# Tom94/practical-path-guiding

Hardware: AMD Instinct MI355X
Metric: Msamples/s (higher is better)
Workload: dtype f32; 1 GPU; room-720p (kitchen-class STAND-IN for the KITCHEN scene, 1397784 Lambertian triangles), 1280x720, 1 spp/pass, 614 passes, improved preset; headline_scene=False, parallelism=tiles1

## Files before the change

### include/ppg_testhooks.h

```cpp
#ifndef PPG_TESTHOOKS_H
#define PPG_TESTHOOKS_H

#include <stdint.h>

#ifdef __cplusplus
extern "C" {
#endif

int ppg_debug_build_bvh(const float *positions, const uint32_t *indices, uint32_t n_triangles, float pad_abs, int32_t max_leaf,
                        void *nodes_out, uint32_t nodes_cap, uint32_t *n_nodes, uint32_t *order_out);

struct ppg_rfilter;
int ppg_debug_rfilter_table(const struct ppg_rfilter *f, float table[32], float *radius, int32_t *border);

struct ppg_ctx;
int ppg_debug_set_defer_depth(struct ppg_ctx *ctx, int32_t depth);

#ifdef __cplusplus
}
#endif
#endif
```

### practical-path-guiding_amd/csrc/ppg_hip.hip

```cpp
#include <hip/hip_runtime.h>

#include <cstring>
#include <map>
#include <mutex>
#include <set>

#include <rocprim/rocprim.hpp>

#include <algorithm>
#include <atomic>
#include <chrono>
#include <cmath>
#include <cstdio>
#include <cstring>
#include <functional>
#include <limits>
#include <map>
#include <memory>
#include <string>
#include <vector>

#include "../../include/ppg.h"
#include "../../include/ppg_testhooks.h"
#include "ppg_kernels.h"
// ... 120 lines not shown
            if (debugAlloc) fprintf(stderr, "[ppg alloc] hipMalloc %zu MiB -> %s (cache holds %zu MiB)\n", want >> 20, e == hipSuccess ? "ok" : "FAILED: cache released", g_blockCache.held >> 20);
            if (e != hipSuccess) {
                (void)hipGetLastError();
                g_blockCache.trim();
                e = hipMalloc(&np, want);
                if (e != hipSuccess) return e;
            }
            got = want;
            (void)hipMemsetAsync(np, 0, want, g_ctxStream);
        }
        if (keep && p && cap) e = hipMemcpyAsync(np, p, cap * sizeof(T), hipMemcpyDeviceToDevice, g_ctxStream);
        if (keep && p && cap && !g_ctxStream) (void)hipStreamSynchronize(nullptr);
        if (p) g_blockCache.give(p, bytes);
        p = np; bytes = got; cap = got / sizeof(T);
        return e;
    }
};

struct HostSNode {
    int axis = 0;
    uint32_t child[2] = {0, 0};
    bool isLeaf() const { return child[0] == 0; }
};

int parseEnum(const char *s, const char *dflt, std::initializer_list<const char *> names) {
    std::string v = s ? s : dflt;
    int i = 0;
    for (const char *n : names) {
        if (v == n) return i;
        ++i;
    }
    return -1;
}

struct BvhBuilder {
    const float *pos; const uint32_t *idx;
    std::vector<uint32_t> order;
    std::vector<float> bmin, bmax, cent;
    std::vector<BvhNode> nodes;
    float pad;
    int maxLeaf = 4;

    struct Box { float lo[3], hi[3]; };
    static Box empty() { Box b; for (int a = 0; a < 3; ++a) { b.lo[a] = INFINITY; b.hi[a] = -INFINITY; } return b; }
    static void grow(Box &b, const float *lo, const float *hi) { for (int a = 0; a < 3; ++a) { b.lo[a] = std::min(b.lo[a], lo[a]); b.hi[a] = std::max(b.hi[a], hi[a]); } }
    static float area(const Box &b) { float d[3] = {b.hi[0] - b.lo[0], b.hi[1] - b.lo[1], b.hi[2] - b.lo[2]}; if (d[0] < 0) return 0; return 2 * (d[0] * d[1] + d[1] * d[2] + d[2] * d[0]); }

    Box boundsOf(int first, int count) const {
        Box b = empty();
        for (int i = first; i < first + count; ++i) grow(b, &bmin[3 * order[i]], &bmax[3 * order[i]]);
        return b;
    }

    void build(int first, int count, int &ref, int &n, Box &box) {
        box = boundsOf(first, count);
        if (count <= maxLeaf) { ref = first; n = count; return; }
        Box cb = empty();
        for (int i = first; i < first + count; ++i) grow(cb, &cent[3 * order[i]], &cent[3 * order[i]]);
        int bestAxis = -1, bestSplit = -1; float bestCost = INFINITY;
        const int NB = 16;
        for (int a = 0; a < 3; ++a) {
            float ext = cb.hi[a] - cb.lo[a];
            if (!(ext > 0)) continue;
            Box bb[NB]; int bc[NB];
            for (int k = 0; k < NB; ++k) { bb[k] = empty(); bc[k] = 0; }
            for (int i = first; i < first + count; ++i) {
                int k = std::min(NB - 1, (int)((cent[3 * order[i] + a] - cb.lo[a]) / ext * NB));
                grow(bb[k], &bmin[3 * order[i]], &bmax[3 * order[i]]); bc[k]++;
            }
            float la[NB]; int lc[NB]; Box acc = empty(); int c = 0;
            for (int k = 0; k < NB; ++k) { if (bc[k]) grow(acc, bb[k].lo, bb[k].hi); c += bc[k]; la[k] = area(acc); lc[k] = c; }
            acc = empty(); c = 0;
            for (int k = NB - 1; k > 0; --k) {
                if (bc[k]) grow(acc, bb[k].lo, bb[k].hi); c += bc[k];
                if (lc[k - 1] == 0 || c == 0) continue;
                float cost = la[k - 1] * lc[k - 1] + area(acc) * c;
                if (cost < bestCost) { bestCost = cost; bestAxis = a; bestSplit = k; }
            }
        }
        int mid;
        if (bestAxis < 0) {
            mid = first + count / 2;
        } else {
            float ext = cb.hi[bestAxis] - cb.lo[bestAxis], lo = cb.lo[bestAxis];
            auto it = std::partition(order.begin() + first, order.begin() + first + count, [&](uint32_t t) {
                int k = std::min(NB - 1, (int)((cent[3 * t + bestAxis] - lo) / ext * NB));
                return k < bestSplit;
            });
            mid = (int)(it - order.begin());
            if (mid == first || mid == first + count) mid = first + count / 2;
        }
        int me = (int)nodes.size();
        nodes.emplace_back();
        int r0, n0, r1, n1; Box b0, b1;
        build(first, mid - first, r0, n0, b0);
        build(mid, first + count - mid, r1, n1, b1);
        BvhNode &nd = nodes[me];
        for (int a = 0; a < 3; ++a) { nd.lo0[a] = b0.lo[a] - pad; nd.hi0[a] = b0.hi[a] + pad; nd.lo1[a] = b1.lo[a] - pad; nd.hi1[a] = b1.hi[a] + pad; }
        nd.c0 = r0; nd.n0 = n0; nd.c1 = r1; nd.n1 = n1;
        ref = me; n = 0;
    }

    std::vector<Bvh4Node> nodes4;
    struct Ref { int ref, n; float lo[3], hi[3]; };
    static float areaRef(const Ref &r) { float d[3] = {r.hi[0] - r.lo[0], r.hi[1] - r.lo[1], r.hi[2] - r.lo[2]}; return 2 * (d[0] * d[1] + d[1] * d[2] + d[2] * d[0]); }
    void childrenOf(int node2, Ref out[2]) const {
        const BvhNode &nd = nodes[node2];
        out[0].ref = nd.c0; out[0].n = nd.n0; out[1].ref = nd.c1; out[1].n = nd.n1;
        for (int a = 0; a < 3; ++a) { out[0].lo[a] = nd.lo0[a]; out[0].hi[a] = nd.hi0[a]; out[1].lo[a] = nd.lo1[a]; out[1].hi[a] = nd.hi1[a]; }
    }
    int make4(int node2) {
        Ref ch[4]; int m = 2;
        childrenOf(node2, ch);
        if (ch[1].n < 0) m = 1;
        while (m < 4) {
            int pick = -1; float best = -1;
            for (int k = 0; k < m; ++k) if (ch[k].n == 0 && areaRef(ch[k]) > best) { best = areaRef(ch[k]); pick = k; }
            if (pick < 0) break;
            Ref two[2]; childrenOf(ch[pick].ref, two);
            ch[pick] = two[0]; ch[m++] = two[1];
        }
        int me = (int)nodes4.size();
        nodes4.emplace_back();
        Bvh4Node nd;
        for (int k = 0; k < 4; ++k) {
            if (k < m) {
                nd.lox[k] = ch[k].lo[0]; nd.loy[k] = ch[k].lo[1]; nd.loz[k] = ch[k].lo[2];
                nd.hix[k] = ch[k].hi[0]; nd.hiy[k] = ch[k].hi[1]; nd.hiz[k] = ch[k].hi[2];
                if (ch[k].n > 0) nd.child[k] = ~((ch[k].ref << 3) | (ch[k].n - 1));
                else nd.child[k] = make4(ch[k].ref);
            } else {
                nd.lox[k] = nd.loy[k] = nd.loz[k] = 0; nd.hix[k] = nd.hiy[k] = nd.hiz[k] = 0; nd.child[k] = PPG_BVH4_EMPTY;
            }
            nd.pad[k] = 0;
        }
        nodes4[me] = nd;
        return me;
    }

    std::vector<Bvh4QNode> nodes4q;
    static float scaleOf(unsigned int e) { const uint32_t bits = e << 23; float f; memcpy(&f, &bits, 4); return f; }
    void quantise() {
        nodes4q.resize(nodes4.size());
        for (size_t i = 0; i < nodes4.size(); ++i) {
            const Bvh4Node &nd = nodes4[i];
            Bvh4QNode q{};
            const float *lo[3] = {nd.lox, nd.loy, nd.loz}, *hi[3] = {nd.hix, nd.hiy, nd.hiz};
            float org[3];
            unsigned int ex[3], qlo[3] = {0, 0, 0}, qhi[3] = {0, 0, 0};
            for (int a = 0; a < 3; ++a) {
                float mn = INFINITY, mx = -INFINITY;
                for (int k = 0; k < 4; ++k) if (nd.child[k] != PPG_BVH4_EMPTY) { mn = std::min(mn, lo[a][k]); mx = std::max(mx, hi[a][k]); }
                if (!(mn <= mx)) { mn = 0; mx = 0; }
                org[a] = mn;
                int x = 0;
                (void)std::frexp((double)(mx - mn) / 255.0, &x);
                int e = std::max(64, std::min(154, x + 127));
                for (;;) {
                    const float s = scaleOf((unsigned int)e);
                    bool ok = true;
                    unsigned int wl = 0, wh = 0;
                    for (int k = 0; k < 4 && ok; ++k) {
                        if (nd.child[k] == PPG_BVH4_EMPTY) { wl |= 255u << (8 * k); continue; }
                        long ql = (long)std::floor(((double)lo[a][k] - (double)mn) / (double)s), qh = (long)std::ceil(((double)hi[a][k] - (double)mn) / (double)s);
                        ql = std::max(0l, std::min(255l, ql)); qh = std::max(0l, qh);
                        auto below = [&](long qq) { return mn + (float)qq * s <= lo[a][k] && (double)mn + (double)qq * (double)s <= (double)lo[a][k]; };
                        auto above = [&](long qq) { return mn + (float)qq * s >= hi[a][k] && (double)mn + (double)qq * (double)s >= (double)hi[a][k]; };
                        while (ql > 0 && !below(ql)) --ql;
                        while (qh <= 255 && !above(qh)) ++qh;
                        if (qh > 255 || !below(ql)) { ok = false; break; }
                        wl |= (unsigned int)ql << (8 * k); wh |= (unsigned int)qh << (8 * k);
                    }
                    if (ok) { qlo[a] = wl; qhi[a] = wh; break; }
                    if (++e > 154) { e = 154; qlo[a] = 0; qhi[a] = 0xffffffffu; break; }
                }
                ex[a] = (unsigned int)e;
            }
            q.ox = org[0]; q.oy = org[1]; q.oz = org[2];
            q.exps = ex[0] | (ex[1] << 8) | (ex[2] << 16);
            q.qlox = qlo[0]; q.qloy = qlo[1]; q.qloz = qlo[2]; q.qhix = qhi[0]; q.qhiy = qhi[1]; q.qhiz = qhi[2];
            for (int k = 0; k < 4; ++k) q.child[k] = nd.child[k];
            nodes4q[i] = q;
        }
    }

    std::vector<float> topCut;
    void buildTopCut() {
        struct Ent { float lo[3], hi[3]; int ref; };
        auto childrenOfQ = [&](int node, Ent out[4]) {
// ... 3 lines not shown
            for (int k = 0; k < 4; ++k) {
                if (q.child[k] == PPG_BVH4_EMPTY) continue;
                const int sh = 8 * k;
                Ent e;
                e.lo[0] = q.ox + (float)((q.qlox >> sh) & 255u) * sx; e.lo[1] = q.oy + (float)((q.qloy >> sh) & 255u) * sy; e.lo[2] = q.oz + (float)((q.qloz >> sh) & 255u) * sz;
                e.hi[0] = q.ox + (float)((q.qhix >> sh) & 255u) * sx; e.hi[1] = q.oy + (float)((q.qhiy >> sh) & 255u) * sy; e.hi[2] = q.oz + (float)((q.qhiz >> sh) & 255u) * sz;
                e.ref = q.child[k];
                out[m++] = e;
            }
            return m;
        };
        std::vector<Ent> cut;
        {
            Ent ch[4];
            const int m = nodes4q.empty() ? 0 : childrenOfQ(0, ch);
            for (int k = 0; k < m; ++k) cut.push_back(ch[k]);
        }
        auto areaOf = [](const Ent &e) { const float d[3] = {e.hi[0] - e.lo[0], e.hi[1] - e.lo[1], e.hi[2] - e.lo[2]}; return d[0] * d[1] + d[1] * d[2] + d[2] * d[0]; };
        for (;;) {
            int pick = -1; float best = -1;
            for (size_t k = 0; k < cut.size(); ++k) if (cut[k].ref >= 0 && areaOf(cut[k]) > best) { best = areaOf(cut[k]); pick = (int)k; }
            if (pick < 0) break;
            Ent ch[4];
            const int m = childrenOfQ(cut[(size_t)pick].ref, ch);
            if (cut.size() - 1 + (size_t)m > 64) break;
            cut.erase(cut.begin() + pick);
            for (int k = 0; k < m; ++k) cut.push_back(ch[k]);
        }
        topCut.assign(8 * cut.size(), 0.0f);
        for (size_t k = 0; k < cut.size(); ++k) {
            float *o = &topCut[8 * k];
            o[0] = cut[k].lo[0]; o[1] = cut[k].lo[1]; o[2] = cut[k].lo[2]; memcpy(o + 3, &cut[k].ref, 4);
            o[4] = cut[k].hi[0]; o[5] = cut[k].hi[1]; o[6] = cut[k].hi[2];
        }
    }

    void run(const float *positions, const uint32_t *indices, uint32_t nTris, float padAbs) {
        runTree(positions, indices, nTris, padAbs);
        buildTopCut();
    }
    void runTree(const float *positions, const uint32_t *indices, uint32_t nTris, float padAbs) {
        pos = positions; idx = indices; pad = padAbs;
        order.resize(nTris); bmin.resize(3 * (size_t)nTris); bmax.resize(3 * (size_t)nTris); cent.resize(3 * (size_t)nTris);
        for (uint32_t t = 0; t < nTris; ++t) {
            order[t] = t;
            for (int a = 0; a < 3; ++a) {
                float v0 = pos[3 * idx[3 * t] + a], v1 = pos[3 * idx[3 * t + 1] + a], v2 = pos[3 * idx[3 * t + 2] + a];
                bmin[3 * t + a] = std::min(v0, std::min(v1, v2)); bmax[3 * t + a] = std::max(v0, std::max(v1, v2));
                cent[3 * t + a] = 0.5f * (bmin[3 * t + a] + bmax[3 * t + a]);
            }
        }
        nodes.clear();
        nodes.reserve(nTris);
        int ref, n; Box b;
        nodes.emplace_back();
        if (nTris == 0) {
            nodes4.assign(1, Bvh4Node{});
            for (int k = 0; k < 4; ++k) nodes4[0].child[k] = PPG_BVH4_EMPTY;
            quantise();
            return;
        }
        if (nTris <= 4) {
            BvhNode &nd = nodes[0];
            Box bb = boundsOf(0, (int)nTris);
            for (int a = 0; a < 3; ++a) { nd.lo0[a] = bb.lo[a] - pad; nd.hi0[a] = bb.hi[a] + pad; nd.lo1[a] = 0; nd.hi1[a] = 0; }
            nd.c0 = 0; nd.n0 = (int)nTris; nd.c1 = 0; nd.n1 = -1;
            nodes4.clear(); make4(0); quantise();
            return;
        }
        nodes.pop_back();
        build(0, (int)nTris, ref, n, b);
        nodes4.clear(); nodes4.reserve(nodes.size() / 2 + 1);
        make4(0);
        quantise();
    }
};

struct KernelTimer {
    struct Rec { hipEvent_t a, b; int id; uint64_t units; };
    std::vector<std::string> names;
    std::vector<double> ms;
    std::vector<uint64_t> launches, units;
    std::vector<Rec> pending;
    std::vector<hipEvent_t> pool;
    bool enabled = false;
    int idOf(const char *n) {
        for (size_t i = 0; i < names.size(); ++i) if (names[i] == n) return (int)i;
        names.push_back(n); ms.push_back(0); launches.push_back(0); units.push_back(0);
        return (int)names.size() - 1;
    }
    hipEvent_t ev() { if (!pool.empty()) { hipEvent_t e = pool.back(); pool.pop_back(); return e; } hipEvent_t e; (void)hipEventCreate(&e); return e; }
    void resolve() {
        for (auto &r : pending) {
            (void)hipEventSynchronize(r.b);
            float t = 0; (void)hipEventElapsedTime(&t, r.a, r.b);
            ms[r.id] += t; launches[r.id]++; units[r.id] += r.units;
            pool.push_back(r.a); pool.push_back(r.b);
        }
        pending.clear();
    }
    void reset() { resolve(); for (size_t i = 0; i < ms.size(); ++i) { ms[i] = 0; launches[i] = 0; units[i] = 0; } }
};

}

struct GroupLaunch { unsigned int firstPass, groupPasses, stridePasses, slot0, slotStride; bool wholeFilm; unsigned int addCount; bool groupsDone = true; bool exchange = false; };

struct ppg_ctx {
    int nee = 0, sampleCombination = 1, spatialFilter = 0, directionalFilter = 0, loss = 0, budgetType = 1;
    int sdTreeMaxMemory = -1, sTreeThreshold = 12000, sppPerPass = 4, rrDepth = 5, maxDepth = -1;
    float dTreeThreshold = 0.01f, bsdfSamplingFraction = 0.5f, budget = 300.0f;
    bool dumpSDTree = false, strictNormals = false, hideEmitters = false;
    uint64_t seed = 0;
    int device = 0;
    std::string dumpPrefix, error;
    hipStream_t stream = nullptr;
    hipStream_t stream2 = nullptr;
    hipEvent_t evFork = nullptr, evJoin = nullptr;
    hipStream_t stream3 = nullptr;
    hipEvent_t evTreeFork = nullptr, evSplatDone = nullptr, evAdamDone = nullptr;
    bool treePending = false;
    void joinTree() {
        if (!treePending) return;
        (void)hipStreamWaitEvent(stream, evSplatDone, 0);
        (void)hipStreamWaitEvent(stream, evAdamDone, 0);
        treePending = false;
    }
    void quiesce() {
        joinTree();
// ... 1907 lines not shown
    r2 = dx * dx + dy * dy + dz * dz;
    ctx->scene.bsphere = make_float4(c[0], c[1], c[2], ppg_max(PPG_EPSILON, std::sqrt(r2) * 1.5f));
}

int ppg_set_scene(ppg_ctx *ctx, const ppg_scene *s) {
    if (!s || !s->materials || (s->n_triangles == 0 && s->n_spheres == 0) ||
        (s->n_triangles > 0 && (!s->positions || !s->indices || !s->tri_material || !s->tri_emitter))) {
        ctx->error = "incomplete scene";
        return PPG_ERR_INVALID;
    }
    HIP_CHECK(hipSetDevice(ctx->device));
    ctx->quiesce();
    for (uint32_t t = 0; t < s->n_triangles; ++t) {
        if (s->tri_material[t] >= s->n_materials || s->tri_emitter[t] >= (int32_t)s->n_emitters) { ctx->error = "index out of range"; return PPG_ERR_INVALID; }
        if (s->materials[s->tri_material[t]].type < 0 || s->materials[s->tri_material[t]].type > PPG_BSDF_LAST) { ctx->error = "unsupported BSDF type"; return PPG_ERR_INVALID; }
        for (int k = 0; k < 3; ++k) if (s->indices[3 * t + k] >= s->n_vertices) { ctx->error = "vertex index out of range"; return PPG_ERR_INVALID; }
    }
    std::vector<int> emitterSphere(s->n_emitters, -1);
    if (s->n_spheres) {
        if (!s->spheres) { ctx->error = "spheres: n_spheres > 0 but no array"; return PPG_ERR_INVALID; }
        std::vector<int> users(s->n_emitters, 0);
        for (uint32_t t = 0; t < s->n_triangles; ++t) if (s->tri_emitter[t] >= 0) users[s->tri_emitter[t]] = 1;
        for (uint32_t k = 0; k < s->n_spheres; ++k) {
            const ppg_sphere &sp = s->spheres[k];
            if (!(sp.radius > 0)) { ctx->error = "sphere: radius must be > 0"; return PPG_ERR_INVALID; }
            if (sp.material >= s->n_materials || sp.emitter >= (int32_t)s->n_emitters) { ctx->error = "index out of range"; return PPG_ERR_INVALID; }
            if (s->materials[sp.material].type < 0 || s->materials[sp.material].type > PPG_BSDF_LAST) { ctx->error = "unsupported BSDF type"; return PPG_ERR_INVALID; }
            if (sp.emitter >= 0 && users[sp.emitter]++) { ctx->error = "sphere: its emitter is shared with another shape"; return PPG_ERR_INVALID; }
            if (sp.emitter >= 0) emitterSphere[sp.emitter] = (int)k;
        }
    }
    float mn[3] = {INFINITY, INFINITY, INFINITY}, mx[3] = {-INFINITY, -INFINITY, -INFINITY};
    for (size_t t = 0; t < 3 * (size_t)s->n_triangles; ++t)
        for (int a = 0; a < 3; ++a) { float v = s->positions[3 * s->indices[t] + a]; mn[a] = ppg_min(mn[a], v); mx[a] = ppg_max(mx[a], v); }
    for (uint32_t k = 0; k < s->n_spheres; ++k)
        for (int a = 0; a < 3; ++a) { mn[a] = ppg_min(mn[a], s->spheres[k].center[a] - s->spheres[k].radius); mx[a] = ppg_max(mx[a], s->spheres[k].center[a] + s->spheres[k].radius); }
    const float eps = 1e-3f;
    for (int a = 0; a < 3; ++a) {
        ctx->geomMin[a] = mn[a] - ((mx[a] - mn[a]) * eps + eps);
        ctx->geomMax[a] = mx[a] + ((mx[a] - ctx->geomMin[a]) * eps + eps);
    }
    sceneBox(ctx, s->camera.camera_to_world);
    float ext = 0;
    for (int a = 0; a < 3; ++a) ext = std::max(ext, mx[a] - mn[a]);
    if (!(ext < 1e9f)) { ctx->error = "scene extent of 1e9 units or more (or not finite)"; return PPG_ERR_INVALID; }
    BvhBuilder bb;
    const float padRel = ctx->tuneBvhPad;
    bb.maxLeaf = ctx->tuneBvhLeaf;
    bb.run(s->positions, s->indices, s->n_triangles, padRel * ext + 1e-30f);
    std::vector<float4> tris(3 * (size_t)s->n_triangles), nrm, accel(3 * (size_t)s->n_triangles);
    if (s->normals) nrm.resize(tris.size());
    for (uint32_t k = 0; k < s->n_triangles; ++k) {
        uint32_t t = bb.order[k];
        {
            const float *A = s->positions + 3 * s->indices[3 * t], *B = s->positions + 3 * s->indices[3 * t + 1], *C = s->positions + 3 * s->indices[3 * t + 2];
            static const int waldModulo[4] = {1, 2, 0, 1};
            const float b[3] = {C[0] - A[0], C[1] - A[1], C[2] - A[2]}, c[3] = {B[0] - A[0], B[1] - A[1], B[2] - A[2]};
            const float N[3] = {c[1] * b[2] - c[2] * b[1], c[2] * b[0] - c[0] * b[2], c[0] * b[1] - c[1] * b[0]};
            int kk = 0;
            for (int j = 0; j < 3; j++) if (ppg_abs(N[j]) > ppg_abs(N[kk])) kk = j;
            const int u = waldModulo[kk], v = waldModulo[kk + 1];
            const float n_k = N[kk], denom = b[u] * c[v] - b[v] * c[u];
            float n_u = 0, n_v = 0, n_d = 0, a_u = 0, a_v = 0, b_nu = 0, b_nv = 0, c_nu = 0, c_nv = 0;
            if (denom == 0) {
                kk = 3;
            } else {
                n_u = N[u] / n_k; n_v = N[v] / n_k;
                n_d = (A[0] * N[0] + A[1] * N[1] + A[2] * N[2]) / n_k;
                b_nu = b[u] / denom; b_nv = -b[v] / denom;
                a_u = A[u]; a_v = A[v];
                c_nu = c[v] / denom; c_nv = -c[u] / denom;
            }
            accel[3 * k + 0] = make_float4(n_u, n_v, n_d, __builtin_bit_cast(float, kk));
            accel[3 * k + 1] = make_float4(a_u, a_v, b_nu, b_nv);
            accel[3 * k + 2] = make_float4(c_nu, c_nv, 0.0f, __builtin_bit_cast(float, (int)t));
        }
        for (int v = 0; v < 3; ++v) {
            const float *p = s->positions + 3 * s->indices[3 * t + v];
            float w = v == 0 ? __builtin_bit_cast(float, (int)s->tri_material[t]) : (v == 1 ? __builtin_bit_cast(float, (int)s->tri_emitter[t]) : __builtin_bit_cast(float, (int)t));
            tris[3 * k + v] = make_float4(p[0], p[1], p[2], w);
            if (s->normals) { const float *n = s->normals + 3 * s->indices[3 * t + v]; nrm[3 * k + v] = make_float4(n[0], n[1], n[2], 0); }
        }
    }
    std::vector<float4> mats(PPG_MAT_STRIDE * (size_t)s->n_materials), ems(std::max<uint32_t>(1, s->n_emitters));
    ctx->fullMaterials = false;
    bool hasNull = false;
    for (uint32_t i = 0; i < s->n_materials; ++i) {
        ppg_material m = s->materials[i];
        if (m.type == PPG_BSDF_DIFFUSE && m.flags == PPG_MAT_TWOSIDED) { m.type = PPG_BSDF_TWOSIDED_DIFFUSE; m.flags = 0; }
        if (m.type == PPG_BSDF_TWOSIDED_DIFFUSE) m.flags &= ~PPG_MAT_TWOSIDED;
        if (m.type == PPG_BSDF_MIRROR) for (int c = 0; c < 3; ++c) { m.eta[c] = 0.0f; m.k[c] = 1.0f; }
        if (m.type == PPG_BSDF_ROUGHCONDUCTOR || m.type == PPG_BSDF_ROUGHDIELECTRIC || m.type == PPG_BSDF_ROUGHPLASTIC) m.alpha = ppg_max(m.alpha, 1e-4f);
        if ((m.type == PPG_BSDF_PLASTIC || m.type == PPG_BSDF_DIELECTRIC || m.type == PPG_BSDF_THINDIELECTRIC || m.type == PPG_BSDF_ROUGHDIELECTRIC) && !(m.eta[0] > 0)) { ctx->error = "plastic / dielectric need eta[0] = intIOR / extIOR > 0"; return PPG_ERR_INVALID; }
        float fdrInt = m.type == PPG_BSDF_PLASTIC ? ppg_fresnel_diffuse_reflectance(1 / m.eta[0]) : 0.0f;
        if (m.type == PPG_BSDF_ROUGHPLASTIC) {
            if (m.rtrans < 0 || (uint32_t)m.rtrans >= s->n_rtrans || !s->rtrans || s->rtrans_samples < 2) { ctx->error = "roughplastic: material.rtrans is not a slice of scene.rtrans"; return PPG_ERR_INVALID; }
            if (!(m.eta[0] > 0)) { ctx->error = "plastic / dielectric need eta[0] = intIOR / extIOR > 0"; return PPG_ERR_INVALID; }
            fdrInt = 1 - s->rtrans[(size_t)m.rtrans * (s->rtrans_samples + 1) + s->rtrans_samples];
        } else m.rtrans = 0;
        if (m.type > PPG_BSDF_MIRROR || m.flags != 0) ctx->fullMaterials = true;
        if (m.type == PPG_BSDF_THINDIELECTRIC || (m.flags & PPG_MAT_MASK)) hasNull = true;
        mats[PPG_MAT_STRIDE * i + 0] = make_float4(m.reflectance[0], m.reflectance[1], m.reflectance[2], (float)m.type);
        mats[PPG_MAT_STRIDE * i + 1] = make_float4(m.specular[0], m.specular[1], m.specular[2], m.alpha);
        mats[PPG_MAT_STRIDE * i + 2] = make_float4(m.eta[0], m.eta[1], m.eta[2], __builtin_bit_cast(float, m.flags));
        mats[PPG_MAT_STRIDE * i + 3] = make_float4(m.k[0], m.k[1], m.k[2], fdrInt);
        mats[PPG_MAT_STRIDE * i + 4] = make_float4(m.opacity[0], m.opacity[1], m.opacity[2], __builtin_bit_cast(float, m.rtrans));
        {
            const uint32_t ta = m.texture & 0xffffu, tb = m.texture >> 16;
            if (ta > s->n_textures || tb > s->n_textures || (m.texture && !s->textures)) { ctx->error = "material.texture: index out of range"; return PPG_ERR_INVALID; }
            if (ta && m.type != PPG_BSDF_DIFFUSE && m.type != PPG_BSDF_TWOSIDED_DIFFUSE && m.type != PPG_BSDF_PLASTIC && m.type != PPG_BSDF_ROUGHPLASTIC) {
                ctx->error = "material.texture: only the diffuse reflectance of diffuse / plastic / roughplastic can carry a bitmap"; return PPG_ERR_INVALID;
            }
            if (m.texture) ctx->fullMaterials = true;
            mats[PPG_MAT_STRIDE * i + 5] = make_float4(__builtin_bit_cast(float, m.texture), 0.0f, 0.0f, 0.0f);
        }
    }
    for (uint32_t k = 0; k < s->n_spheres; ++k)
        if (s->materials[s->spheres[k].material].texture) { ctx->error = "sphere: textured BSDFs are only supported on triangle meshes"; return PPG_ERR_INVALID; }
    ctx->scene.uvs = nullptr; ctx->scene.textures = nullptr;
    if (s->texcoords) {
        std::vector<float2> uv(3 * (size_t)s->n_triangles);
        for (uint32_t k = 0; k < s->n_triangles; ++k) {
            const uint32_t t = bb.order[k];
            for (int v = 0; v < 3; ++v) { const float *q = s->texcoords + 2 * (size_t)s->indices[3 * t + v]; uv[3 * (size_t)k + v] = make_float2(q[0], q[1]); }
        }
        HIP_CHECK(ctx->d_uvs.reserve(uv.size()));
        HIP_CHECK(hipMemcpy(ctx->d_uvs.p, uv.data(), uv.size() * sizeof(float2), hipMemcpyHostToDevice));
        ctx->scene.uvs = ctx->d_uvs.p;
    }
// ... 239 lines not shown
        ctx->pathsReady = true;
    }
    return PPG_OK;
}

int ppg_set_shard(ppg_ctx *ctx, int32_t rank, int32_t world, int32_t tile_size) {
    (void)hipSetDevice(ctx->device);
    ctx->quiesce();
    if (world < 1 || rank < 0 || rank >= world || tile_size < 1) { ctx->error = "bad shard"; return PPG_ERR_INVALID; }
    if (world > 1 && ctx->filtered && !ctx->footHook) { ctx->error = kShardedFilter; return PPG_ERR_INVALID; }
    ctx->shardRank = rank; ctx->shardWorld = world; ctx->tileSize = tile_size;
    ctx->pathsReady = false;
    if (ctx->haveScene) {
        int rc = allocPaths(ctx);
        if (rc) return rc;
        if ((rc = allocFilm(ctx))) return rc;
        if ((rc = presizeRounds(ctx))) return rc;
        ctx->pathsReady = true;
    }
    return PPG_OK;
}

#define NEED_SCENE (void)hipSetDevice(ctx->device); StreamScope scope_(ctx->stream); if (!ctx->haveScene) { ctx->error = "no scene"; return PPG_ERR_STATE; }
#define NEED_TREE (void)hipSetDevice(ctx->device); StreamScope scope_(ctx->stream); if (!ctx->treeAlive) { ctx->error = "render not begun"; return PPG_ERR_STATE; } ctx->joinTree();

int ppg_begin_render(ppg_ctx *ctx) { NEED_SCENE return beginRender(ctx); }
int ppg_begin_iteration(ppg_ctx *ctx, int32_t is_final) { NEED_TREE return beginIteration(ctx, is_final != 0); }
int ppg_set_final(ppg_ctx *ctx, int32_t is_final) { ctx->isFinalIter = is_final != 0; return PPG_OK; }
int ppg_set_do_nee(ppg_ctx *ctx, int32_t do_nee) { ctx->doNee = do_nee != 0; return PPG_OK; }
int ppg_render_passes_nostat(ppg_ctx *ctx, int32_t n) { NEED_TREE return renderPassesNoStat(ctx, n); }
int ppg_finish_passes(ppg_ctx *ctx, ppg_pass_stats *st) { NEED_TREE return finishPasses(ctx, st); }
int ppg_render_passes(ppg_ctx *ctx, int32_t n, ppg_pass_stats *st) {
    NEED_TREE
    int rc = renderPassesNoStat(ctx, n);
    if (rc && rc != PPG_ERR_CANCELLED) return rc;
    int rc2 = finishPasses(ctx, st);
    return rc ? rc : rc2;
}
int ppg_build_sdtree(ppg_ctx *ctx, ppg_tree_stats *st) { NEED_TREE return buildSDTree(ctx, st); }
int ppg_end_iteration(ppg_ctx *ctx) { NEED_TREE return endIteration(ctx); }
int ppg_end_render(ppg_ctx *ctx) { NEED_TREE return endRender(ctx); }
int ppg_cancel(ppg_ctx *ctx) { ctx->cancelled.store(true); return PPG_OK; }
int ppg_debug_build_bvh(const float *positions, const uint32_t *indices, uint32_t n_triangles, float pad_abs, int32_t max_leaf,
                        void *nodes_out, uint32_t nodes_cap, uint32_t *n_nodes, uint32_t *order_out) {
    if (!positions || !indices || !n_nodes || n_triangles == 0) return PPG_ERR_INVALID;
    BvhBuilder bb;
    bb.maxLeaf = std::max(1, std::min(8, (int)max_leaf));
    bb.run(positions, indices, n_triangles, pad_abs);
    *n_nodes = (uint32_t)bb.nodes4q.size();
    if (nodes_out) memcpy(nodes_out, bb.nodes4q.data(), std::min<size_t>(nodes_cap, bb.nodes4q.size()) * sizeof(Bvh4QNode));
    if (order_out) memcpy(order_out, bb.order.data(), (size_t)n_triangles * sizeof(uint32_t));
    return PPG_OK;
}
static int rfilterTable(const ppg_rfilter *f, float table[32], float *radius, int32_t *border, std::string &err) {
    const int type = f->type;
    float r = 0.0f;
    switch (type) {
    case PPG_RFILTER_BOX:
        if (!(std::isfinite(f->radius) && f->radius > 0.0f)) { err = "box filter: radius must be positive"; return PPG_ERR_INVALID; }
        r = f->radius + 1e-5f; break;
    case PPG_RFILTER_TENT: r = 1.0f; break;
    case PPG_RFILTER_GAUSSIAN:
        if (!(std::isfinite(f->stddev) && f->stddev > 0.0f)) { err = "gaussian filter: stddev must be positive"; return PPG_ERR_INVALID; }
        r = 4 * f->stddev; break;
    case PPG_RFILTER_MITCHELL:
        if (!(std::isfinite(f->B) && std::isfinite(f->C))) { err = "mitchell filter: B and C must be finite"; return PPG_ERR_INVALID; }
        r = 2.0f; break;
    case PPG_RFILTER_CATMULLROM: r = 2.0f; break;
    case PPG_RFILTER_LANCZOS:
        if (f->lobes < 1) { err = "lanczos filter: lobes must be >= 1"; return PPG_ERR_INVALID; }
        r = (float)f->lobes; break;
    default: err = "unknown reconstruction filter type"; return PPG_ERR_INVALID;
    }
    const float stddev = f->stddev, B = f->B, C = f->C;
    auto mitchell = [](float x, float B, float C) {
        x = std::fabs(x);
        const float x2 = x * x, x3 = x2 * x;
        if (x < 1) return 1.0f / 6.0f * ((12 - 9 * B - 6 * C) * x3 + (-18 + 12 * B + 6 * C) * x2 + (6 - 2 * B));
        if (x < 2) return 1.0f / 6.0f * ((-B - 6 * C) * x3 + (6 * B + 30 * C) * x2 + (-12 * B - 48 * C) * x + (8 * B + 24 * C));
        return 0.0f;
    };
    auto eval = [&](float x) -> float {
        switch (type) {
        case PPG_RFILTER_BOX: return std::fabs(x) <= r ? 1.0f : 0.0f;
        case PPG_RFILTER_TENT: return std::max(0.0f, 1.0f - std::fabs(x / r));
        case PPG_RFILTER_GAUSSIAN: {
            const float alpha = -1.0f / (2.0f * stddev * stddev);
            return std::max(0.0f, (float)std::exp((double)(alpha * x * x)) - (float)std::exp((double)(alpha * r * r)));
        }
        case PPG_RFILTER_MITCHELL: return mitchell(x, B, C);
        case PPG_RFILTER_CATMULLROM: return mitchell(x, 0.0f, 0.5f);
        default: {
            x = std::fabs(x);
            if (x < 1e-4f) return 1.0f;
            if (x > r) return 0.0f;
            const float x1 = (float)(M_PI * (double)x), x2 = x1 / r;
            return (std::sin(x1) * std::sin(x2)) / (x1 * x2);
        }
        }
    };
    float sum = 0.0f;
    for (int i = 0; i < 31; ++i) { table[i] = eval((r * (float)i) / 31); sum += table[i]; }
    table[31] = 0.0f;
    sum *= 2 * r / 31;
    const float normalization = 1.0f / sum;
    for (int i = 0; i < 31; ++i) table[i] *= normalization;
// ... 362 lines not shown
```

Baseline: 231.3 Msamples/s.

## Rebuild BVH with sweep SAH, insertion reoptimisation and cost-optimal 4-wide collapse

Replaces the binned-SAH binary build with full sweep SAH for small ranges (binning for larger ones), builds down to single-triangle leaves, runs batched node reinsertion to lower SAH, and then collapses to BVH4 with a dynamic-programming cost model that picks leaf sizes and child cuts. The goal is fewer node visits and triangle tests per ray in the traversal kernels that dominate path tracing. In exchange, host build time goes up considerably (sorts and priority-queue searches over 1.4M triangles). Host-side debug stats and a CPU trace hook are also added.

Measured after the change: 250.4 Msamples/s (median of 6 runs). 8.2% higher.

```diff
diff --git a/include/ppg_testhooks.h b/include/ppg_testhooks.h
--- a/include/ppg_testhooks.h
+++ b/include/ppg_testhooks.h
@@ -10,6 +10,20 @@
 int ppg_debug_build_bvh(const float *positions, const uint32_t *indices, uint32_t n_triangles, float pad_abs, int32_t max_leaf,
                         void *nodes_out, uint32_t nodes_cap, uint32_t *n_nodes, uint32_t *order_out);
 
+struct ppg_bvh_stats {
+    uint32_t n_nodes, n_leaves, depth, n_binary_nodes;
+    uint32_t leaf_hist[9];
+    uint32_t reserved;
+    double sa_interior, sa_leaf, sa_tris;
+    double build_seconds;
+};
+int ppg_debug_bvh_stats(const float *positions, const uint32_t *indices, uint32_t n_triangles, float pad_abs, int32_t max_leaf,
+                        struct ppg_bvh_stats *out);
+
+int ppg_debug_bvh_trace(const float *positions, const uint32_t *indices, uint32_t n_triangles, float pad_abs, int32_t max_leaf,
+                        const float *rays, uint32_t n_rays, float *t_out, int32_t *orig_out, uint32_t *steps_out, uint32_t *tests_out,
+                        uint32_t *max_stack);
+
 struct ppg_rfilter;
 int ppg_debug_rfilter_table(const struct ppg_rfilter *f, float table[32], float *radius, int32_t *border);
 
diff --git a/practical-path-guiding_amd/csrc/ppg_hip.hip b/practical-path-guiding_amd/csrc/ppg_hip.hip
--- a/practical-path-guiding_amd/csrc/ppg_hip.hip
+++ b/practical-path-guiding_amd/csrc/ppg_hip.hip
@@ -196,11 +196,44 @@
         return b;
     }
 
-    void build(int first, int count, int &ref, int &n, Box &box) {
-        box = boundsOf(first, count);
-        if (count <= maxLeaf) { ref = first; n = count; return; }
-        Box cb = empty();
-        for (int i = first; i < first + count; ++i) grow(cb, &cent[3 * order[i]], &cent[3 * order[i]]);
+    struct N2 {
+        float lo[3], hi[3];
+        int parent, c0, c1;
+        int tri;
+        int first, count;
+    };
+    std::vector<N2> t2;
+    static float areaN(const N2 &n) { const float d[3] = {n.hi[0] - n.lo[0], n.hi[1] - n.lo[1], n.hi[2] - n.lo[2]}; return 2 * (d[0] * d[1] + d[1] * d[2] + d[2] * d[0]); }
+    static float areaU(const N2 &p, const N2 &q) {
+        float d[3];
+        for (int a = 0; a < 3; ++a) d[a] = std::max(p.hi[a], q.hi[a]) - std::min(p.lo[a], q.lo[a]);
+        return 2 * (d[0] * d[1] + d[1] * d[2] + d[2] * d[0]);
+    }
+    static constexpr int SWEEP = 64;
+    std::vector<uint32_t> swCur, swBest;
+    std::vector<float> swArea;
+    int sweepSplit(int first, int count) {
+        swCur.resize((size_t)count); swBest.resize((size_t)count); swArea.resize((size_t)count);
+        float bestCost = INFINITY; int bestI = -1;
+        for (int a = 0; a < 3; ++a) {
+            std::copy(order.begin() + first, order.begin() + first + count, swCur.begin());
+            std::sort(swCur.begin(), swCur.end(), [&](uint32_t x, uint32_t y) { const float cx = cent[3 * x + a], cy = cent[3 * y + a]; return cx < cy || (cx == cy && x < y); });
+            Box acc = empty();
+            for (int i = count - 1; i >= 1; --i) { grow(acc, &bmin[3 * swCur[i]], &bmax[3 * swCur[i]]); swArea[i] = area(acc); }
+            acc = empty();
+            bool better = false;
+            for (int i = 1; i < count; ++i) {
+                grow(acc, &bmin[3 * swCur[i - 1]], &bmax[3 * swCur[i - 1]]);
+                const float cost = area(acc) * i + swArea[i] * (count - i);
+                if (cost < bestCost) { bestCost = cost; bestI = i; better = true; }
+            }
+            if (better) swBest.swap(swCur);
+        }
+        if (bestI < 0) return first + count / 2;
+        std::copy(swBest.begin(), swBest.end(), order.begin() + first);
+        return first + bestI;
+    }
+    int binnedSplit(int first, int count, const Box &cb) {
         int bestAxis = -1, bestSplit = -1; float bestCost = INFINITY;
         const int NB = 16;
         for (int a = 0; a < 3; ++a) {
@@ -222,63 +255,211 @@
                 if (cost < bestCost) { bestCost = cost; bestAxis = a; bestSplit = k; }
             }
         }
+        if (bestAxis < 0) return first + count / 2;
+        float ext = cb.hi[bestAxis] - cb.lo[bestAxis], lo = cb.lo[bestAxis];
+        auto it = std::partition(order.begin() + first, order.begin() + first + count, [&](uint32_t t) {
+            int k = std::min(NB - 1, (int)((cent[3 * t + bestAxis] - lo) / ext * NB));
+            return k < bestSplit;
+        });
+        int mid = (int)(it - order.begin());
+        if (mid == first || mid == first + count) mid = first + count / 2;
+        return mid;
+    }
+    int build2(int first, int count, int parent) {
+        const int me = (int)t2.size();
+        t2.emplace_back();
+        {
+            N2 &n = t2[(size_t)me];
+            const Box b = boundsOf(first, count);
+            for (int a = 0; a < 3; ++a) { n.lo[a] = b.lo[a]; n.hi[a] = b.hi[a]; }
+            n.parent = parent; n.c0 = n.c1 = -1; n.tri = (int)order[first]; n.first = first; n.count = count;
+        }
+        if (count == 1) return me;
+        Box cb = empty();
+        for (int i = first; i < first + count; ++i) grow(cb, &cent[3 * order[i]], &cent[3 * order[i]]);
         int mid;
-        if (bestAxis < 0) {
-            mid = first + count / 2;
-        } else {
-            float ext = cb.hi[bestAxis] - cb.lo[bestAxis], lo = cb.lo[bestAxis];
-            auto it = std::partition(order.begin() + first, order.begin() + first + count, [&](uint32_t t) {
-                int k = std::min(NB - 1, (int)((cent[3 * t + bestAxis] - lo) / ext * NB));
-                return k < bestSplit;
-            });
-            mid = (int)(it - order.begin());
-            if (mid == first || mid == first + count) mid = first + count / 2;
-        }
-        int me = (int)nodes.size();
-        nodes.emplace_back();
-        int r0, n0, r1, n1; Box b0, b1;
-        build(first, mid - first, r0, n0, b0);
-        build(mid, first + count - mid, r1, n1, b1);
-        BvhNode &nd = nodes[me];
-        for (int a = 0; a < 3; ++a) { nd.lo0[a] = b0.lo[a] - pad; nd.hi0[a] = b0.hi[a] + pad; nd.lo1[a] = b1.lo[a] - pad; nd.hi1[a] = b1.hi[a] + pad; }
-        nd.c0 = r0; nd.n0 = n0; nd.c1 = r1; nd.n1 = n1;
-        ref = me; n = 0;
-    }
-
+        if (!(cb.hi[0] > cb.lo[0]) && !(cb.hi[1] > cb.lo[1]) && !(cb.hi[2] > cb.lo[2])) mid = first + count / 2;
+        else mid = count <= SWEEP ? sweepSplit(first, count) : binnedSplit(first, count, cb);
+        const int l = build2(first, mid - first, me), r = build2(mid, first + count - mid, me);
+        t2[(size_t)me].c0 = l; t2[(size_t)me].c1 = r;
+        return me;
+    }
+
+    void refit(int v) {
+        for (; v >= 0; v = t2[(size_t)v].parent) {
+            N2 &n = t2[(size_t)v];
+            const N2 &p = t2[(size_t)n.c0], &q = t2[(size_t)n.c1];
+            bool same = true;
+            for (int a = 0; a < 3; ++a) {
+                const float lo = std::min(p.lo[a], q.lo[a]), hi = std::max(p.hi[a], q.hi[a]);
+                same = same && lo == n.lo[a] && hi == n.hi[a];
+                n.lo[a] = lo; n.hi[a] = hi;
+            }
+            if (same) break;
+        }
+    }
+    void replaceChild(int p, int was, int now) { N2 &n = t2[(size_t)p]; if (n.c0 == was) n.c0 = now; else n.c1 = now; t2[(size_t)now].parent = p; }
+    typedef std::pair<float, int> QEnt;
+    std::vector<QEnt> heap;
+    int findTarget(int x) {
+        auto later = [](const QEnt &p, const QEnt &q) { return p.first > q.first || (p.first == q.first && p.second > q.second); };
+        const float ax = areaN(t2[(size_t)x]);
+        float best = INFINITY; int bestNode = -1;
+        heap.clear();
+        heap.push_back(QEnt(0.0f, 0));
+        while (!heap.empty()) {
+            std::pop_heap(heap.begin(), heap.end(), later);
+            const QEnt e = heap.back();
+            heap.pop_back();
+            if (e.first + ax >= best && bestNode >= 0) break;
+            const N2 &v = t2[(size_t)e.second];
+            const float total = e.first + areaU(v, t2[(size_t)x]);
+            if (e.second != 0 && (total < best || bestNode < 0)) { best = total; bestNode = e.second; }
+            const float below = total - areaN(v);
+            if (v.c0 >= 0 && (below + ax < best || bestNode < 0)) {
+                heap.push_back(QEnt(below, v.c0)); std::push_heap(heap.begin(), heap.end(), later);
+                heap.push_back(QEnt(below, v.c1)); std::push_heap(heap.begin(), heap.end(), later);
+            }
+        }
+        return bestNode;
+    }
+    void insertAt(int x, int spare) {
+        const int b = findTarget(x), bp = t2[(size_t)b].parent;
+        replaceChild(bp, b, spare);
+        N2 &f = t2[(size_t)spare];
+        f.c0 = b; f.c1 = x;
+        t2[(size_t)b].parent = spare; t2[(size_t)x].parent = spare;
+        for (int a = 0; a < 3; ++a) { f.lo[a] = std::min(t2[(size_t)b].lo[a], t2[(size_t)x].lo[a]); f.hi[a] = std::max(t2[(size_t)b].hi[a], t2[(size_t)x].hi[a]); }
+        refit(bp);
+    }
+    bool movable(int n) const { return n > 0 && t2[(size_t)n].c0 >= 0 && t2[(size_t)n].parent > 0; }
+    void reinsert(int n) {
+        const int p = t2[(size_t)n].parent, g = t2[(size_t)p].parent;
+        const int s = t2[(size_t)p].c0 == n ? t2[(size_t)p].c1 : t2[(size_t)p].c0;
+        replaceChild(g, p, s);
+        refit(g);
+        int l = t2[(size_t)n].c0, r = t2[(size_t)n].c1;
+        if (areaN(t2[(size_t)l]) < areaN(t2[(size_t)r])) std::swap(l, r);
+        insertAt(l, n);
+        insertAt(r, p);
+    }
+    static constexpr int REOPT_PART = 100, REOPT_BATCHES = 8;
+    void reoptimise() {
+        if (t2.size() < 16) return;
+        std::vector<QEnt> cand;
+        for (int batch = 0; batch < REOPT_BATCHES; ++batch) {
+            cand.clear();
+            for (int v = 1; v < (int)t2.size(); ++v) {
+                if (!movable(v)) continue;
+                const float a = areaN(t2[(size_t)v]), a0 = areaN(t2[(size_t)t2[(size_t)v].c0]), a1 = areaN(t2[(size_t)t2[(size_t)v].c1]);
+                const float tiny = 1e-30f;
+                const float prio = a * (a / std::max(std::min(a0, a1), tiny)) * (a / std::max(0.5f * (a0 + a1), tiny));
+                if (prio == prio) cand.push_back(QEnt(prio, v));
+            }
+            const size_t k = std::min(cand.size(), std::max<size_t>(1, t2.size() / (2 * REOPT_PART)));
+            auto first = [](const QEnt &p, const QEnt &q) { return p.first > q.first || (p.first == q.first && p.second < q.second); };
+            std::partial_sort(cand.begin(), cand.begin() + (long)k, cand.end(), first);
+            for (size_t i = 0; i < k; ++i) if (movable(cand[i].second)) reinsert(cand[i].second);
+        }
+    }
+
+    std::vector<int> pre;
+    void layout() {
+        std::vector<uint32_t> fresh;
+        fresh.reserve(order.size());
+        pre.clear(); pre.reserve(t2.size());
+        std::vector<int> stack(1, 0);
+        while (!stack.empty()) {
+            const int v = stack.back();
+            stack.pop_back();
+            pre.push_back(v);
+            N2 &n = t2[(size_t)v];
+            if (n.c0 < 0) { n.first = (int)fresh.size(); n.count = 1; fresh.push_back((uint32_t)n.tri); }
+            else { stack.push_back(n.c1); stack.push_back(n.c0); }
+        }
+        for (size_t i = pre.size(); i-- > 0;) {
+            N2 &n = t2[(size_t)pre[i]];
+            if (n.c0 >= 0) { n.first = t2[(size_t)n.c0].first; n.count = t2[(size_t)n.c0].count + t2[(size_t)n.c1].count; }
+        }
+        order.swap(fresh);
+    }
+
+    static constexpr double C_NODE = 1.0, C_LEAF = 0.25, C_TRI = 0.25;
+    struct Cost4 { double k[4]; };
+    std::vector<Cost4> cost;
+    std::vector<unsigned char> asLeaf;
+    double paddedArea(const N2 &n) const {
+        const double d[3] = {(double)n.hi[0] - n.lo[0] + 2.0 * pad, (double)n.hi[1] - n.lo[1] + 2.0 * pad, (double)n.hi[2] - n.lo[2] + 2.0 * pad};
+        return 2 * (d[0] * d[1] + d[1] * d[2] + d[2] * d[0]);
+    }
+    void collapse() {
+        cost.resize(t2.size()); asLeaf.assign(t2.size(), 0);
+        for (size_t i = pre.size(); i-- > 0;) {
+            const int v = pre[i];
+            const N2 &n = t2[(size_t)v];
+            const double A = paddedArea(n);
+            Cost4 &c = cost[(size_t)v];
+            if (n.c0 < 0) { c.k[0] = A * (C_LEAF + C_TRI); c.k[1] = c.k[2] = c.k[3] = INFINITY; asLeaf[(size_t)v] = 1; continue; }
+            const Cost4 &l = cost[(size_t)n.c0], &r = cost[(size_t)n.c1];
+            double cut = INFINITY;
+            for (int k = 2; k <= 4; ++k) {
+                double best = INFINITY;
+                for (int j = 1; j < k; ++j) best = std::min(best, l.k[j - 1] + r.k[k - j - 1]);
+                c.k[k - 1] = best;
+                cut = std::min(cut, best);
+            }
+            const double node = A * C_NODE + cut, leaf = n.count <= maxLeaf ? A * (C_LEAF + C_TRI * n.count) : INFINITY;
+            asLeaf[(size_t)v] = leaf <= node;
+            c.k[0] = std::min(leaf, node);
+        }
+    }
+    void cut4(int v, int k, int *ch, int &m) const {
+        if (k == 1) { ch[m++] = v; return; }
+        const N2 &n = t2[(size_t)v];
+        const Cost4 &l = cost[(size_t)n.c0], &r = cost[(size_t)n.c1];
+        int bj = 1;
+        for (int j = 2; j < k; ++j) if (l.k[j - 1] + r.k[k - j - 1] < l.k[bj - 1] + r.k[k - bj - 1]) bj = j;
+        cut4(n.c0, bj, ch, m);
+        cut4(n.c1, k - bj, ch, m);
+    }
     std::vector<Bvh4Node> nodes4;
-    struct Ref { int ref, n; float lo[3], hi[3]; };
-    static float areaRef(const Ref &r) { float d[3] = {r.hi[0] - r.lo[0], r.hi[1] - r.lo[1], r.hi[2] - r.lo[2]}; return 2 * (d[0] * d[1] + d[1] * d[2] + d[2] * d[0]); }
-    void childrenOf(int node2, Ref out[2]) const {
-        const BvhNode &nd = nodes[node2];
-        out[0].ref = nd.c0; out[0].n = nd.n0; out[1].ref = nd.c1; out[1].n = nd.n1;
-        for (int a = 0; a < 3; ++a) { out[0].lo[a] = nd.lo0[a]; out[0].hi[a] = nd.hi0[a]; out[1].lo[a] = nd.lo1[a]; out[1].hi[a] = nd.hi1[a]; }
-    }
-    int make4(int node2) {
-        Ref ch[4]; int m = 2;
-        childrenOf(node2, ch);
-        if (ch[1].n < 0) m = 1;
-        while (m < 4) {
-            int pick = -1; float best = -1;
-            for (int k = 0; k < m; ++k) if (ch[k].n == 0 && areaRef(ch[k]) > best) { best = areaRef(ch[k]); pick = k; }
-            if (pick < 0) break;
-            Ref two[2]; childrenOf(ch[pick].ref, two);
-            ch[pick] = two[0]; ch[m++] = two[1];
-        }
-        int me = (int)nodes4.size();
+    int emit4(int v) {
+        int ch[4], m = 0, bk = 2;
+        for (int k = 3; k <= 4; ++k) if (cost[(size_t)v].k[k - 1] < cost[(size_t)v].k[bk - 1]) bk = k;
+        cut4(v, bk, ch, m);
+        const int me = (int)nodes4.size();
         nodes4.emplace_back();
         Bvh4Node nd;
         for (int k = 0; k < 4; ++k) {
             if (k < m) {
-                nd.lox[k] = ch[k].lo[0]; nd.loy[k] = ch[k].lo[1]; nd.loz[k] = ch[k].lo[2];
-                nd.hix[k] = ch[k].hi[0]; nd.hiy[k] = ch[k].hi[1]; nd.hiz[k] = ch[k].hi[2];
-                if (ch[k].n > 0) nd.child[k] = ~((ch[k].ref << 3) | (ch[k].n - 1));
-                else nd.child[k] = make4(ch[k].ref);
+                const N2 &c = t2[(size_t)ch[k]];
+                nd.lox[k] = c.lo[0] - pad; nd.loy[k] = c.lo[1] - pad; nd.loz[k] = c.lo[2] - pad;
+                nd.hix[k] = c.hi[0] + pad; nd.hiy[k] = c.hi[1] + pad; nd.hiz[k] = c.hi[2] + pad;
+                if (asLeaf[(size_t)ch[k]]) nd.child[k] = ~((c.first << 3) | (c.count - 1));
+                else nd.child[k] = emit4(ch[k]);
             } else {
                 nd.lox[k] = nd.loy[k] = nd.loz[k] = 0; nd.hix[k] = nd.hiy[k] = nd.hiz[k] = 0; nd.child[k] = PPG_BVH4_EMPTY;
             }
             nd.pad[k] = 0;
         }
-        nodes4[me] = nd;
+        nodes4[(size_t)me] = nd;
+        return me;
+    }
+    int emit2(int v) {
+        const int me = (int)nodes.size();
+        nodes.emplace_back();
+        BvhNode nd;
+        const int ch[2] = {t2[(size_t)v].c0, t2[(size_t)v].c1};
+        int ref[2], cnt[2];
+        for (int k = 0; k < 2; ++k) {
+            const N2 &c = t2[(size_t)ch[k]];
+            if (asLeaf[(size_t)ch[k]]) { ref[k] = c.first; cnt[k] = c.count; }
+            else { ref[k] = emit2(ch[k]); cnt[k] = 0; }
+            float *lo = k ? nd.lo1 : nd.lo0, *hi = k ? nd.hi1 : nd.hi0;
+            for (int a = 0; a < 3; ++a) { lo[a] = c.lo[a] - pad; hi[a] = c.hi[a] + pad; }
+        }
+        nd.c0 = ref[0]; nd.n0 = cnt[0]; nd.c1 = ref[1]; nd.n1 = cnt[1];
+        nodes[(size_t)me] = nd;
         return me;
     }
 
@@ -388,7 +569,6 @@
         }
         nodes.clear();
         nodes.reserve(nTris);
-        int ref, n; Box b;
         nodes.emplace_back();
         if (nTris == 0) {
             nodes4.assign(1, Bvh4Node{});
@@ -401,16 +581,49 @@
             Box bb = boundsOf(0, (int)nTris);
             for (int a = 0; a < 3; ++a) { nd.lo0[a] = bb.lo[a] - pad; nd.hi0[a] = bb.hi[a] + pad; nd.lo1[a] = 0; nd.hi1[a] = 0; }
             nd.c0 = 0; nd.n0 = (int)nTris; nd.c1 = 0; nd.n1 = -1;
-            nodes4.clear(); make4(0); quantise();
+            Bvh4Node n4{};
+            for (int k = 0; k < 4; ++k) n4.child[k] = PPG_BVH4_EMPTY;
+            n4.lox[0] = nd.lo0[0]; n4.loy[0] = nd.lo0[1]; n4.loz[0] = nd.lo0[2]; n4.hix[0] = nd.hi0[0]; n4.hiy[0] = nd.hi0[1]; n4.hiz[0] = nd.hi0[2];
+            n4.child[0] = ~((0 << 3) | ((int)nTris - 1));
+            nodes4.assign(1, n4);
+            quantise();
             return;
         }
         nodes.pop_back();
-        build(0, (int)nTris, ref, n, b);
-        nodes4.clear(); nodes4.reserve(nodes.size() / 2 + 1);
-        make4(0);
+        t2.clear(); t2.reserve(2 * (size_t)nTris);
+        build2(0, (int)nTris, -1);
+        reoptimise();
+        layout();
+        collapse();
+        nodes4.clear(); nodes4.reserve(t2.size() / 4 + 1);
+        emit4(0);
+        emit2(0);
         quantise();
     }
 };
+
+static void triAccelLoad(const float *A, const float *B, const float *C, int orig, float4 out[3]) {
+    static const int waldModulo[4] = {1, 2, 0, 1};
+    const float b[3] = {C[0] - A[0], C[1] - A[1], C[2] - A[2]}, c[3] = {B[0] - A[0], B[1] - A[1], B[2] - A[2]};
+    const float N[3] = {c[1] * b[2] - c[2] * b[1], c[2] * b[0] - c[0] * b[2], c[0] * b[1] - c[1] * b[0]};
+    int kk = 0;
+    for (int j = 0; j < 3; j++) if (ppg_abs(N[j]) > ppg_abs(N[kk])) kk = j;
+    const int u = waldModulo[kk], v = waldModulo[kk + 1];
+    const float n_k = N[kk], denom = b[u] * c[v] - b[v] * c[u];
+    float n_u = 0, n_v = 0, n_d = 0, a_u = 0, a_v = 0, b_nu = 0, b_nv = 0, c_nu = 0, c_nv = 0;
+    if (denom == 0) {
+        kk = 3;
+    } else {
+        n_u = N[u] / n_k; n_v = N[v] / n_k;
+        n_d = (A[0] * N[0] + A[1] * N[1] + A[2] * N[2]) / n_k;
+        b_nu = b[u] / denom; b_nv = -b[v] / denom;
+        a_u = A[u]; a_v = A[v];
+        c_nu = c[v] / denom; c_nv = -c[u] / denom;
+    }
+    out[0] = make_float4(n_u, n_v, n_d, __builtin_bit_cast(float, kk));
+    out[1] = make_float4(a_u, a_v, b_nu, b_nv);
+    out[2] = make_float4(c_nu, c_nv, 0.0f, __builtin_bit_cast(float, orig));
+}
 
 struct KernelTimer {
     struct Rec { hipEvent_t a, b; int id; uint64_t units; };
@@ -2424,29 +2637,7 @@
     if (s->normals) nrm.resize(tris.size());
     for (uint32_t k = 0; k < s->n_triangles; ++k) {
         uint32_t t = bb.order[k];
-        {
-            const float *A = s->positions + 3 * s->indices[3 * t], *B = s->positions + 3 * s->indices[3 * t + 1], *C = s->positions + 3 * s->indices[3 * t + 2];
-            static const int waldModulo[4] = {1, 2, 0, 1};
-            const float b[3] = {C[0] - A[0], C[1] - A[1], C[2] - A[2]}, c[3] = {B[0] - A[0], B[1] - A[1], B[2] - A[2]};
-            const float N[3] = {c[1] * b[2] - c[2] * b[1], c[2] * b[0] - c[0] * b[2], c[0] * b[1] - c[1] * b[0]};
-            int kk = 0;
-            for (int j = 0; j < 3; j++) if (ppg_abs(N[j]) > ppg_abs(N[kk])) kk = j;
-            const int u = waldModulo[kk], v = waldModulo[kk + 1];
-            const float n_k = N[kk], denom = b[u] * c[v] - b[v] * c[u];
-            float n_u = 0, n_v = 0, n_d = 0, a_u = 0, a_v = 0, b_nu = 0, b_nv = 0, c_nu = 0, c_nv = 0;
-            if (denom == 0) {
-                kk = 3;
-            } else {
-                n_u = N[u] / n_k; n_v = N[v] / n_k;
-                n_d = (A[0] * N[0] + A[1] * N[1] + A[2] * N[2]) / n_k;
-                b_nu = b[u] / denom; b_nv = -b[v] / denom;
-                a_u = A[u]; a_v = A[v];
-                c_nu = c[v] / denom; c_nv = -c[u] / denom;
-            }
-            accel[3 * k + 0] = make_float4(n_u, n_v, n_d, __builtin_bit_cast(float, kk));
-            accel[3 * k + 1] = make_float4(a_u, a_v, b_nu, b_nv);
-            accel[3 * k + 2] = make_float4(c_nu, c_nv, 0.0f, __builtin_bit_cast(float, (int)t));
-        }
+        triAccelLoad(s->positions + 3 * s->indices[3 * t], s->positions + 3 * s->indices[3 * t + 1], s->positions + 3 * s->indices[3 * t + 2], (int)t, &accel[3 * k]);
         for (int v = 0; v < 3; ++v) {
             const float *p = s->positions + 3 * s->indices[3 * t + v];
             float w = v == 0 ? __builtin_bit_cast(float, (int)s->tri_material[t]) : (v == 1 ? __builtin_bit_cast(float, (int)s->tri_emitter[t]) : __builtin_bit_cast(float, (int)t));
@@ -2792,6 +2983,151 @@
     if (order_out) memcpy(order_out, bb.order.data(), (size_t)n_triangles * sizeof(uint32_t));
     return PPG_OK;
 }
+static void decodeChildBox(const Bvh4QNode &q, int k, float lo[3], float hi[3]) {
+    const float s[3] = {BvhBuilder::scaleOf(q.exps & 255u), BvhBuilder::scaleOf((q.exps >> 8) & 255u), BvhBuilder::scaleOf((q.exps >> 16) & 255u)};
+    const float org[3] = {q.ox, q.oy, q.oz};
+    const unsigned int ql[3] = {q.qlox, q.qloy, q.qloz}, qh[3] = {q.qhix, q.qhiy, q.qhiz};
+    for (int a = 0; a < 3; ++a) {
+        lo[a] = org[a] + (float)((ql[a] >> (8 * k)) & 255u) * s[a];
+        hi[a] = org[a] + (float)((qh[a] >> (8 * k)) & 255u) * s[a];
+    }
+}
+int ppg_debug_bvh_stats(const float *positions, const uint32_t *indices, uint32_t n_triangles, float pad_abs, int32_t max_leaf, ppg_bvh_stats *out) {
+    if (!positions || !indices || !out || n_triangles == 0) return PPG_ERR_INVALID;
+    BvhBuilder bb;
+    bb.maxLeaf = std::max(1, std::min(8, (int)max_leaf));
+    const auto t0 = std::chrono::steady_clock::now();
+    bb.run(positions, indices, n_triangles, pad_abs);
+    const auto t1 = std::chrono::steady_clock::now();
+    memset(out, 0, sizeof(*out));
+    out->build_seconds = std::chrono::duration<double>(t1 - t0).count();
+    out->n_nodes = (uint32_t)bb.nodes4q.size();
+    out->n_binary_nodes = (uint32_t)bb.nodes.size();
+    auto areaOf = [](const float lo[3], const float hi[3]) {
+        const double d[3] = {(double)hi[0] - lo[0], (double)hi[1] - lo[1], (double)hi[2] - lo[2]};
+        return d[0] < 0 || d[1] < 0 || d[2] < 0 ? 0.0 : 2 * (d[0] * d[1] + d[1] * d[2] + d[2] * d[0]);
+    };
+    double rootArea = 0;
+    {
+        float lo[3] = {INFINITY, INFINITY, INFINITY}, hi[3] = {-INFINITY, -INFINITY, -INFINITY};
+        for (int k = 0; k < 4; ++k) {
+            if (bb.nodes4q[0].child[k] == PPG_BVH4_EMPTY) continue;
+            float l[3], h[3];
+            decodeChildBox(bb.nodes4q[0], k, l, h);
+            for (int a = 0; a < 3; ++a) { lo[a] = std::min(lo[a], l[a]); hi[a] = std::max(hi[a], h[a]); }
+        }
+        rootArea = areaOf(lo, hi);
+    }
+    const double inv = rootArea > 0 ? 1.0 / rootArea : 0.0;
+    std::vector<std::pair<int, uint32_t>> stack(1, {0, 1u});
+    while (!stack.empty()) {
+        const std::pair<int, uint32_t> e = stack.back();
+        stack.pop_back();
+        out->depth = std::max(out->depth, e.second);
+        const Bvh4QNode &q = bb.nodes4q[(size_t)e.first];
+        for (int k = 0; k < 4; ++k) {
+            if (q.child[k] == PPG_BVH4_EMPTY) continue;
+            float l[3], h[3];
+            decodeChildBox(q, k, l, h);
+            const double a = areaOf(l, h) * inv;
+            if (q.child[k] >= 0) { out->sa_interior += a; stack.push_back({q.child[k], e.second + 1}); }
+            else {
+                const int cnt = (~q.child[k] & 7) + 1;
+                out->sa_leaf += a; out->sa_tris += a * cnt; out->n_leaves++; out->leaf_hist[cnt]++;
+            }
+        }
+    }
+    return PPG_OK;
+}
+int ppg_debug_bvh_trace(const float *positions, const uint32_t *indices, uint32_t n_triangles, float pad_abs, int32_t max_leaf, const float *rays,
+                        uint32_t n_rays, float *t_out, int32_t *orig_out, uint32_t *steps_out, uint32_t *tests_out, uint32_t *max_stack) {
+    if (!positions || !indices || n_triangles == 0 || (n_rays && !rays)) return PPG_ERR_INVALID;
+    BvhBuilder bb;
+    bb.maxLeaf = std::max(1, std::min(8, (int)max_leaf));
+    bb.run(positions, indices, n_triangles, pad_abs);
+    std::vector<float4> accel(3 * (size_t)n_triangles);
+    for (uint32_t k = 0; k < n_triangles; ++k) {
+        const uint32_t t = bb.order[k];
+        triAccelLoad(positions + 3 * indices[3 * t], positions + 3 * indices[3 * t + 1], positions + 3 * indices[3 * t + 2], (int)t, &accel[3 * (size_t)k]);
+    }
+    auto bits = [](unsigned int u) { float f; memcpy(&f, &u, 4); return f; };
+    uint32_t deepest = 0;
+    std::vector<int> stack;
+    for (uint32_t r = 0; r < n_rays; ++r) {
+        const float *R = rays + 8 * (size_t)r;
+        const float o[3] = {R[0], R[1], R[2]}, d[3] = {R[4], R[5], R[6]}, mint = R[3], maxt = R[7];
+        const float id[3] = {d[0] == 0.0f ? 1e30f : 1.0f / d[0], d[1] == 0.0f ? 1e30f : 1.0f / d[1], d[2] == 0.0f ? 1e30f : 1.0f / d[2]};
+        float bestT = INFINITY;
+        int bestOrig = 0x7fffffff;
+        bool found = false;
+        uint32_t steps = 0, tests = 0;
+        stack.clear();
+        int cur = 0;
+        for (;;) {
+            if (cur >= 0) {
+                ++steps;
+                const Bvh4QNode &q = bb.nodes4q[(size_t)cur];
+                const float tlim = std::min(maxt, bestT);
+                const float org[3] = {q.ox, q.oy, q.oz};
+                const unsigned int ql[3] = {q.qlox, q.qloy, q.qloz}, qh[3] = {q.qhix, q.qhiy, q.qhiz};
+                float os[3], ids[3];
+                for (int a = 0; a < 3; ++a) {
+                    const unsigned int e = (q.exps >> (8 * a)) & 255u;
+                    os[a] = (o[a] - org[a]) * bits((254u - e) << 23);
+                    ids[a] = id[a] * bits(e << 23);
+                }
+                float ts[4]; int cs[4], m = 0;
+                for (int k = 0; k < 4; ++k) {
+                    float n = mint, f = INFINITY;
+                    for (int a = 0; a < 3; ++a) {
+                        const float lo = (float)((ql[a] >> (8 * k)) & 255u), hi = (float)((qh[a] >> (8 * k)) & 255u);
+                        const float tn = ((id[a] < 0 ? hi : lo) - os[a]) * ids[a], tf = ((id[a] < 0 ? lo : hi) - os[a]) * ids[a];
+                        n = std::max(n, tn); f = std::min(f, tf);
+                    }
+                    f = std::min(f * 1.0000008f, tlim);
+                    const bool hit = n <= f && q.child[k] != PPG_BVH4_EMPTY;
+                    ts[k] = hit ? n : INFINITY; cs[k] = q.child[k];
+                    m += hit ? 1 : 0;
+                }
+                auto cswap = [&](int i, int j) { if (ts[i] > ts[j]) { std::swap(ts[i], ts[j]); std::swap(cs[i], cs[j]); } };
+                cswap(0, 1); cswap(2, 3); cswap(0, 2); cswap(1, 3); cswap(1, 2);
+                if (m > 0) {
+                    for (int k = m - 1; k >= 1; --k) stack.push_back(cs[k]);
+                    deepest = std::max<uint32_t>(deepest, (uint32_t)stack.size());
+                    cur = cs[0];
+                    continue;
+                }
+            } else {
+                const int code = ~cur, first = code >> 3, cnt = (code & 7) + 1;
+                for (int qd = first; qd < first + cnt; ++qd) {
+                    ++tests;
+                    const float4 a0 = accel[3 * (size_t)qd], a1 = accel[3 * (size_t)qd + 1], a2 = accel[3 * (size_t)qd + 2];
+                    int k; memcpy(&k, &a0.w, 4);
+                    if ((unsigned int)k > 2u) continue;
+                    const bool k0 = k == 0, k1 = k == 1;
+                    const float o_u = k0 ? o[1] : (k1 ? o[2] : o[0]), o_v = k0 ? o[2] : (k1 ? o[0] : o[1]), o_k = k0 ? o[0] : (k1 ? o[1] : o[2]);
+                    const float d_u = k0 ? d[1] : (k1 ? d[2] : d[0]), d_v = k0 ? d[2] : (k1 ? d[0] : d[1]), d_k = k0 ? d[0] : (k1 ? d[1] : d[2]);
+                    const float t = (a0.z - o_u * a0.x - o_v * a0.y - o_k) / (d_u * a0.x + d_v * a0.y + d_k);
+                    if (t < mint || t > std::min(maxt, bestT)) continue;
+                    const float hu = o_u + t * d_u - a1.x, hv = o_v + t * d_v - a1.y;
+                    const float u = hv * a1.z + hu * a1.w, v = hu * a2.x + hv * a2.y;
+                    if (!(u >= 0 && v >= 0 && u + v <= 1.0f)) continue;
+                    int orig; memcpy(&orig, &a2.w, 4);
+                    if (!found || t < bestT || (t == bestT && orig < bestOrig)) { bestT = t; bestOrig = orig; found = true; }
+                }
+            }
+            if (stack.empty()) break;
+            cur = stack.back();
+            stack.pop_back();
+        }
+        if (t_out) t_out[r] = found ? bestT : INFINITY;
+        if (orig_out) orig_out[r] = found ? bestOrig : -1;
+        if (steps_out) steps_out[r] = steps;
+        if (tests_out) tests_out[r] = tests;
+    }
+    if (max_stack) *max_stack = deepest;
+    return PPG_OK;
+}
 static int rfilterTable(const ppg_rfilter *f, float table[32], float *radius, int32_t *border, std::string &err) {
     const int type = f->type;
     float r = 0.0f;
```
